# marcin119a/vae-los-angeles

Measured on AMD Instinct MI355X. Metric: training samples/sec, MultiModalVAE batch 65536, higher is better.
Workload: dtype bf16

## Files before the change

### include/mmvae_hip.h

```cpp
#ifndef MMVAE_HIP_H
#define MMVAE_HIP_H
#include <stdint.h>

#ifdef __cplusplus
extern "C" {
#endif

#define MMVAE_OK 0
#define MMVAE_ERR_ARG (-1)
#define MMVAE_ERR_DTYPE (-2)

enum { MMVAE_F32 = 0, MMVAE_BF16 = 1 };
enum { MMVAE_PREC_F32 = 0, MMVAE_PREC_BF16 = 1 };
enum { MMVAE_PRO_NONE = 0, MMVAE_PRO_BN_RELU_DROP = 1, MMVAE_PRO_BN_BWD_APPLY = 2 };
enum { MMVAE_EPI_STORE = 0, MMVAE_EPI_RELU_MASK = 1, MMVAE_EPI_BN_BWD = 2, MMVAE_EPI_LOSS_MSE = 3, MMVAE_EPI_LOSS_BCE_LOGIT = 4 };
enum { MMVAE_ACT_NONE = 0, MMVAE_ACT_RELU = 1, MMVAE_ACT_SIGMOID = 2 };

#define MMVAE_TILE 128

int mmvae_abi_version(void);
int mmvae_set_tuning(int32_t key, int32_t value);

typedef struct {
    const float* src; void* dst;
// ... 112 lines not shown
int mmvae_loss_finalize(const double* sums, float beta, float gamma, const float* beta_gamma_dev, float* out5, void* stream);

int mmvae_sigmoid_bwd(int32_t M, int32_t N, const float* g, int64_t ldg, const float* p, int64_t ldpp,
                      void* out, int32_t out_dtype, int64_t ldo, void* stream);

int mmvae_scale_if_needed(void* x, int32_t dtype, int64_t n, const float* scale_dev, void* stream);
#define MMVAE_SCALE_MAX 8
typedef struct { void* x; int64_t n; int32_t dtype; int32_t pad_; } mmvae_scale_item;
int mmvae_scale_many(const mmvae_scale_item* items_host, int32_t n_items, const float* scale_dev, void* stream);

#define MMVAE_CTR_COPIES 16384
int mmvae_noise(uint8_t* mask, int64_t n_mask, float keep_prob, float* eps, int64_t n_eps, uint64_t seed, uint64_t offset,
                uint64_t* offset_dev, int32_t advance, void* stream);
int mmvae_counter_add(uint64_t* counter_dev, uint64_t inc, void* stream);

#define MMVAE_GATHER_MAX 4
typedef struct { const void* src; void* dst; int64_t src_row_stride; int64_t dst_row_stride; int32_t row_bytes; int32_t pad_; } mmvae_gather_item;
int mmvae_gather_rows(const mmvae_gather_item* items_host, int32_t n_items, const int64_t* idx_dev, int32_t rows,
                      int64_t src_rows, void* stream);

int mmvae_rows_to_bf16(const void* src, int32_t src_dtype, int64_t ld_src, void* dst, int64_t ld_dst, int32_t rows, int32_t cols,
                       void* stream);

typedef struct { float* p; const float* g; float* m; float* v; int64_t n; } mmvae_adamw_item;
int mmvae_adamw_step(const mmvae_adamw_item* items_host, int32_t n_items, float lr, float beta1,
                     float beta2, float eps, float weight_decay, float bias_corr1, float bias_corr2, int32_t maximize,
                     uint64_t* step_dev, int32_t advance, const float* lr_dev, void* stream);

#ifdef __cplusplus
}
// ... 3 lines not shown
```

### vae-los-angeles_amd/csrc/elementwise.hip

```cpp
#include <vector>
#include "common.h"
#include "mmvae_hip.h"

namespace mm {

__global__ __launch_bounds__(256) void prep_weights_kernel(const mmvae_prep_item* __restrict__ items) {
    const mmvae_prep_item it = items[blockIdx.y];
    __shared__ float tile[32][33];
    const int tx = threadIdx.x & 31, ty = threadIdx.x >> 5;
    const int tiles_c = (it.dst_cols + 31) / 32, tiles_r = (it.dst_rows + 31) / 32;
    auto put = [&](int r, int c, float v) {
        if (it.dst_dtype == MMVAE_BF16) ((bf16*)it.dst)[(long)r * it.dst_ld + c] = (bf16)v;
        else ((float*)it.dst)[(long)r * it.dst_ld + c] = v;
    };
    for (int t = blockIdx.x; t < tiles_r * tiles_c; t += gridDim.x) {
        const int tr = t / tiles_c, tc = t - tr * tiles_c;
        if (it.transpose) {
#pragma unroll
            for (int k = 0; k < 4; ++k) {
                const int sr = tc * 32 + ty + 8 * k, sc = tr * 32 + tx;
                tile[ty + 8 * k][tx] = (sr < it.src_rows && sc < it.src_cols) ? it.src[(long)sr * it.src_ld + sc] : 0.f;
            }
            __syncthreads();
#pragma unroll
            for (int k = 0; k < 4; ++k) {
                const int r = tr * 32 + ty + 8 * k, c = tc * 32 + tx;
                if (r < it.dst_rows && c < it.dst_cols) put(r, c, tile[tx][ty + 8 * k]);
            }
            __syncthreads();
        } else {
#pragma unroll
            for (int k = 0; k < 4; ++k) {
                const int r = tr * 32 + ty + 8 * k, c = tc * 32 + tx;
                if (r < it.dst_rows && c < it.dst_cols) put(r, c, (r < it.src_rows && c < it.src_cols) ? it.src[(long)r * it.src_ld + c] : 0.f);
            }
        }
    }
}

__global__ __launch_bounds__(256) void bn_finalize_kernel(mmvae_bn_finalize_args a) {
    const int col = blockIdx.x * blockDim.x + threadIdx.x;
    if (col < a.N) {
        const double mean = a.sum[col] / a.M;
        double var = a.sumsq[col] / a.M - mean * mean;
        if (var < 0.0) var = 0.0;
        const float rstd = (float)(1.0 / sqrt(var + (double)a.eps));
        const float sc = a.gamma[col] * rstd;
        a.mean[col] = (float)mean; a.rstd[col] = rstd;
        a.scale[col] = sc; a.shift[col] = a.beta[col] - (float)mean * sc;
        if (a.running_mean) {
            a.running_mean[col] = (1.f - a.momentum) * a.running_mean[col] + a.momentum * (float)mean;
            const double unbiased = var * ((double)a.M / (double)(a.M - 1));
// ... 81 lines not shown
        }
#pragma unroll
        for (int u = 0; u < U; ++u) {
            if (r + u * dr >= (unsigned)M) break;
            float o[V];
#pragma unroll
            for (int e = 0; e < V; ++e) {
                const float xh = (yv[u][e] - mu[e]) * rs[e];
                o[e] = c0[e] * (dv[u][e] - c1[e] - xh * c2[e]);
            }
            store_vec<T, V>(d + (long)rr[u] * ldd + c, o);
        }
    }
}

__global__ __launch_bounds__(256) void embed_table_fwd_kernel(int S, int E, int L, const float* emb, const float* w_mu,
                                                               const float* b_mu, const float* w_lv, const float* b_lv, float* table) {
    for (int i = blockIdx.x * blockDim.x + threadIdx.x; i < S * 2 * L; i += gridDim.x * blockDim.x) {
        const int s = i / (2 * L), j = i % (2 * L);
        const float* w = j < L ? w_mu + (long)j * E : w_lv + (long)(j - L) * E;
        float acc = j < L ? b_mu[j] : b_lv[j - L];
        for (int e = 0; e < E; ++e) acc += emb[(long)s * E + e] * w[e];
        table[i] = acc;
    }
}

__global__ __launch_bounds__(256) void embed_table_bwd_kernel(int S, int E, int L, const float* emb, const float* w_mu,
                                                               const float* w_lv, const float* dTc, int copies, float* d_emb, float* d_w_mu,
                                                               float* d_b_mu, float* d_w_lv, float* d_b_lv) {
    const int L2 = 2 * L;
    extern __shared__ float sm[];
    float* dT = sm;
    float* sE = dT + S * L2;
    float* sW = sE + S * E;
    const int t0 = blockIdx.x * blockDim.x + threadIdx.x, nt = gridDim.x * blockDim.x;
    const int n0 = S * E, n1 = n0 + L2 * E, n2 = n1 + L2;
    auto dst_of = [&](int i) -> float* {
        if (i < n0) return d_emb + i;
        if (i < n1) { const int k = i - n0, j = k / E, e = k - j * E; return j < L ? d_w_mu + (long)j * E + e : d_w_lv + (long)(j - L) * E + e; }
// ... 413 lines not shown
            float sn, cs;
            sincosf(6.283185307179586f * u2, &sn, &cs);
            z[2 * k] = rad * cs; z[2 * k + 1] = rad * sn;
        }
        if (q * 4 + 4 <= n && (((uintptr_t)out & 15) == 0)) *(f32x4*)(out + q * 4) = f32x4{z[0], z[1], z[2], z[3]};
        else for (int k = 0; k < 4; ++k) if (q * 4 + k < n) out[q * 4 + k] = z[k];
}

__device__ __forceinline__ uint64_t ctr_read(const uint64_t* copies, unsigned L) { return copies[L % MMVAE_CTR_COPIES]; }
__device__ __forceinline__ void ctr_advance(uint64_t* copies, unsigned L, unsigned nblocks, uint64_t value) {
    __syncthreads();
    if (threadIdx.x == 0 && threadIdx.y == 0)
        for (unsigned e = L; e < MMVAE_CTR_COPIES; e += nblocks) copies[e] = value;
}

__global__ __launch_bounds__(256) void noise_kernel(uint8_t* mask, long n_mask, float* eps, long n_eps, uint32_t thresh,
                                                    uint64_t seed, uint64_t offset, uint64_t* offset_dev, uint64_t advance, int copies) {
    const uint64_t base = offset_dev ? (copies ? ctr_read(offset_dev, blockIdx.x) : *offset_dev) : 0;
    offset += base;
    const long nqm = (n_mask + 15) / 16, nqe = (n_eps + 3) / 4;
    for (long q = (long)blockIdx.x * blockDim.x + threadIdx.x; q < nqm + nqe; q += (long)gridDim.x * blockDim.x) {
        if (q < nqm) mask_quad(mask, n_mask, q, thresh, seed, offset);
        else randn_quad(eps, n_eps, q - nqm, seed, offset + (uint64_t)nqm * 4);
    }
    if (copies) ctr_advance(offset_dev, blockIdx.x, gridDim.x, base + advance);
}

__global__ void counter_add_kernel(uint64_t* ctr, uint64_t inc) { *ctr += inc; }

struct GatherBatch { mmvae_gather_item it[MMVAE_GATHER_MAX]; int n; };
__global__ __launch_bounds__(256) void gather_rows_kernel(const GatherBatch b, const int64_t* __restrict__ idx, int rows, long src_rows) {
    const int lane = threadIdx.x & 63;
    const long wave0 = ((long)blockIdx.x * blockDim.x + threadIdx.x) >> 6, nwaves = ((long)gridDim.x * blockDim.x) >> 6;
    for (long w = wave0; w < (long)rows * b.n; w += nwaves) {
        const int t = (int)(w / rows), i = (int)(w - (long)t * rows);
        const mmvae_gather_item it = b.it[t];
        long r = idx[i];
        r = r < 0 ? 0 : (r >= src_rows ? src_rows - 1 : r);
        const char* sp = (const char*)it.src + r * it.src_row_stride;
        char* dp = (char*)it.dst + (long)i * it.dst_row_stride;
// ... 79 lines not shown
static inline int grid_for(long items, int per_block = 256, int cap = 2048) {
    long g = (items + per_block - 1) / per_block;
    if (g < 1) g = 1;
    if (g > cap) g = cap;
    return (int)g;
}

}

using namespace mm;

extern "C" int mmvae_abi_version(void) { return 20; }

extern "C" int mmvae_prep_weights(const mmvae_prep_item* items_dev, int32_t n_items, void* stream) {
    if (!items_dev || n_items <= 0) return MMVAE_ERR_ARG;
    hipLaunchKernelGGL(prep_weights_kernel, dim3(160, n_items), dim3(256), 0, (hipStream_t)stream, items_dev);
    MM_CHECK_LAUNCH();
    return 0;
}

extern "C" int mmvae_bn_finalize(const mmvae_bn_finalize_args* a, void* stream) {
    if (!a || !a->sum || !a->sumsq || !a->gamma || !a->beta || !a->mean || !a->rstd || !a->scale || !a->shift) return MMVAE_ERR_ARG;
    if (a->M < 2 || a->N <= 0) return MMVAE_ERR_ARG;
    hipLaunchKernelGGL(bn_finalize_kernel, dim3((a->N + 255) / 256), dim3(256), 0, (hipStream_t)stream, *a);
    MM_CHECK_LAUNCH();
    return 0;
}

extern "C" int mmvae_bn_eval_coeffs(int32_t N, const float* gamma, const float* beta, const float* rm, const float* rv,
                                    float eps, float* scale, float* shift, float* mean, float* rstd, void* stream) {
    if (N <= 0 || !gamma || !beta || !rm || !rv || !scale || !shift) return MMVAE_ERR_ARG;
// ... 187 lines not shown
    }
    hipLaunchKernelGGL(scale_many_kernel, dim3(grid_for(nmax)), dim3(256), 0, (hipStream_t)stream, b, scale_dev);
    MM_CHECK_LAUNCH();
    return 0;
}

extern "C" int mmvae_scale_if_needed(void* x, int32_t dtype, int64_t n, const float* scale_dev, void* stream) {
    if (!x || n <= 0 || !scale_dev) return MMVAE_ERR_ARG;
    const int grid = grid_for(n);
    if (dtype == MMVAE_BF16) hipLaunchKernelGGL(scale_if_needed_kernel<bf16>, dim3(grid), dim3(256), 0, (hipStream_t)stream, (bf16*)x, n, scale_dev);
    else hipLaunchKernelGGL(scale_if_needed_kernel<float>, dim3(grid), dim3(256), 0, (hipStream_t)stream, (float*)x, n, scale_dev);
    MM_CHECK_LAUNCH();
    return 0;
}

extern "C" int mmvae_noise(uint8_t* mask, int64_t n_mask, float keep_prob, float* eps, int64_t n_eps, uint64_t seed,
                           uint64_t offset, uint64_t* offset_dev, int32_t advance, void* stream) {
    if ((n_mask > 0 && (!mask || ((uintptr_t)mask & 15))) || (n_eps > 0 && !eps) || n_mask < 0 || n_eps < 0 || n_mask + n_eps == 0 ||
        keep_prob < 0.f || keep_prob > 1.f || (advance && !offset_dev)) return MMVAE_ERR_ARG;
    const uint64_t used = (uint64_t)((n_mask + 15) / 16 * 4 + (n_eps + 3) / 4);
    const double t = (double)keep_prob * 4294967296.0;
    const uint32_t thresh = t >= 4294967295.0 ? 0xFFFFFFFFu : (uint32_t)t;
    hipLaunchKernelGGL(noise_kernel, dim3(grid_for((n_mask + 15) / 16 + (n_eps + 3) / 4)), dim3(256), 0, (hipStream_t)stream,
                       mask, n_mask, eps, n_eps, thresh, seed, offset, offset_dev, used, advance ? 1 : 0);
    MM_CHECK_LAUNCH();
    return 0;
}

extern "C" int mmvae_gather_rows(const mmvae_gather_item* items_host, int32_t n_items, const int64_t* idx_dev, int32_t rows,
                                 int64_t src_rows, void* stream) {
    if (!items_host || n_items <= 0 || n_items > MMVAE_GATHER_MAX || !idx_dev || rows <= 0 || src_rows <= 0) return MMVAE_ERR_ARG;
    GatherBatch b; b.n = n_items;
    for (int k = 0; k < n_items; ++k) {
        const mmvae_gather_item& it = items_host[k];
        if (!it.src || !it.dst || it.row_bytes <= 0 || it.row_bytes % 4 || it.src_row_stride % 4 || it.dst_row_stride % 4 ||
            ((uintptr_t)it.src & 3) || ((uintptr_t)it.dst & 3)) return MMVAE_ERR_ARG;
        b.it[k] = it;
    }
    const long waves = (long)rows * n_items;
// ... 57 lines not shown
```

### vae-los-angeles_amd/mmvae/_lib.py

```python
import ctypes as C
import os

_HERE = os.path.dirname(os.path.abspath(__file__))
LIB_PATH = os.environ.get("MMVAE_LIB_PATH") or os.path.join(_HERE, "libmmvae_hip.so")
ABI_VERSION = 20

F32, BF16 = 0, 1
PREC_F32, PREC_BF16 = 0, 1
PRO_NONE, PRO_BN_RELU_DROP, PRO_BN_BWD_APPLY = 0, 1, 2
TABLE_COPIES = 8
EPI_STORE, EPI_RELU_MASK, EPI_BN_BWD, EPI_LOSS_MSE, EPI_LOSS_BCE_LOGIT = 0, 1, 2, 3, 4
ACT_NONE, ACT_RELU, ACT_SIGMOID = 0, 1, 2
TILE = 128
TN_GROUP_MAX = 8
CTR_COPIES = 16384

i32, i64, f32, vp = C.c_int32, C.c_int64, C.c_float, C.c_void_p


class PrepItem(C.Structure):
    _fields_ = [("src", vp), ("dst", vp), ("src_rows", i32), ("src_cols", i32), ("src_ld", i64),
                ("dst_rows", i32), ("dst_cols", i32), ("dst_ld", i64), ("transpose", i32), ("dst_dtype", i32)]


# ... 68 lines not shown
                ("sums", vp),
                ("g_a", vp), ("g_a_dtype", i32), ("ld_ga", i64),
                ("g_b", vp), ("g_b_dtype", i32), ("ld_gb", i64), ("grad_b_wrt_logit", i32),
                ("g_c", vp), ("ld_gc", i64),
                ("g_mu", vp), ("g_lv", vp), ("beta_gamma_dev", vp), ("a_dtype", i32), ("b_dtype", i32)]


class GatherItem(C.Structure):
    _fields_ = [("src", vp), ("dst", vp), ("src_row_stride", i64), ("dst_row_stride", i64), ("row_bytes", i32), ("pad_", i32)]


class AdamWItem(C.Structure):
    _fields_ = [("p", vp), ("g", vp), ("m", vp), ("v", vp), ("n", i64)]


_SIGNATURES = {
    "mmvae_set_tuning": [i32, i32],
    "mmvae_prep_weights": [vp, i32, vp],
    "mmvae_gemm_nt": [C.POINTER(GemmNtArgs), vp],
    "mmvae_gemm_tn": [C.POINTER(GemmTnArgs), vp],
    "mmvae_gemm_tn_group": [vp, i32, vp],
    "mmvae_bn_finalize": [C.POINTER(BnFinalizeArgs), vp],
    "mmvae_bn_eval_coeffs": [i32, vp, vp, vp, vp, f32, vp, vp, vp, vp, vp],
    "mmvae_bn_bwd_finalize": [C.POINTER(BnBwdFinalizeArgs), vp],
    "mmvae_bn_bwd_apply": [i32, i32, i32, vp, i64, vp, i64, vp, vp, vp, vp],
    "mmvae_bn_bwd_finalize_apply": [i32, i32, i32, vp, i64, vp, i64, vp, vp, vp, vp, vp, vp, vp, i32, vp],
    "mmvae_embed_table_fwd": [i32, i32, i32, vp, vp, vp, vp, vp, vp, vp],
    "mmvae_embed_table_bwd": [i32, i32, i32, vp, vp, vp, vp, i32, vp, vp, vp, vp, vp, vp],
    "mmvae_fuse_reparam_fwd": [C.POINTER(FuseFwdArgs), vp],
    "mmvae_fuse_reparam_bwd": [C.POINTER(FuseBwdArgs), vp],
    "mmvae_vae_loss": [C.POINTER(LossArgs), vp],
    "mmvae_loss_finalize": [vp, f32, f32, vp, vp, vp],
    "mmvae_gather_rows": [vp, i32, vp, i32, i64, vp],
    "mmvae_rows_to_bf16": [vp, i32, i64, vp, i64, i32, i32, vp],
    "mmvae_sigmoid_bwd": [i32, i32, vp, i64, vp, i64, vp, i32, i64, vp],
    "mmvae_scale_if_needed": [vp, i32, i64, vp, vp],
    "mmvae_scale_many": [C.POINTER(ScaleItem), i32, vp, vp],
    "mmvae_noise": [vp, i64, f32, vp, i64, C.c_uint64, C.c_uint64, vp, i32, vp],
    "mmvae_counter_add": [vp, C.c_uint64, vp],
    "mmvae_adamw_step": [vp, i32, f32, f32, f32, f32, f32, f32, f32, i32, vp, i32, vp, vp],
}
EXPORTED = ["mmvae_abi_version"] + sorted(_SIGNATURES)

_lib = None


class MMVAELibraryError(RuntimeError):
    pass


class MMVAEArgError(RuntimeError):
    """The library refused the arguments (MMVAE_ERR_ARG / MMVAE_ERR_DTYPE) and enqueued nothing (mmvae_hip.h)."""


def load():
    global _lib
    if _lib is not None:
        return _lib
    if not os.path.exists(LIB_PATH):
        raise MMVAELibraryError(
            f"{LIB_PATH} not found: the HIP extension is required (no CPU / eager fallback). "
            "Build it with `python __graft_entry__.py` or `make -C vae-los-angeles_amd/csrc`.")
    lib = C.CDLL(LIB_PATH)
    lib.mmvae_abi_version.restype = C.c_int
    v = lib.mmvae_abi_version()
    if v != ABI_VERSION:
        raise MMVAELibraryError(f"libmmvae_hip.so ABI {v} != binding ABI {ABI_VERSION}; rebuild")
    for name, argtypes in _SIGNATURES.items():
        fn = getattr(lib, name)
        fn.restype = C.c_int
        fn.argtypes = argtypes
    _lib = lib
    return lib


def check(status, what):
    if status in (-1, -2):
        kind = "invalid argument" if status == -1 else "dtype not supported for this precision"
        raise MMVAEArgError(f"{what} failed: {kind}")
    if status != 0:
        raise RuntimeError(f"{what} failed: hipError {status}")
```

### vae-los-angeles_amd/mmvae/engine.py

```python
import os
from dataclasses import dataclass
from typing import NamedTuple, Optional

import torch

from . import ops
from . import _lib as L_
from .ops import (PREC_BF16, PREC_F32, ACT_NONE, ACT_RELU, ACT_SIGMOID, EPI_RELU_MASK, EPI_BN_BWD, DROP_P,
                  ceil_to, act_dtype, Prologue, BnBwdEpilogue, BnBwdFinalize, BnBwdApply)

_PRECISIONS = {"bf16": PREC_BF16, "fp32": PREC_F32, "f32": PREC_F32}
_default_precision = _PRECISIONS[os.environ.get("MMVAE_PRECISION", "bf16").lower()]
_TINY_DW_MAX = 16384


def set_default_precision(name):
    global _default_precision
    _default_precision = _PRECISIONS[name.lower()]


def default_precision():
    return _default_precision


class NoiseSource:

    def __init__(self):
        self._injected = None
# ... 17 lines not shown

    def offset_tensor(self, device):
        t = self._offsets.get(device)
        if t is None:
            t = self._offsets[device] = torch.zeros(L_.CTR_COPIES, dtype=torch.int64, device=device)
        return t

    def state_dict(self, device):
        t = self._offsets.get(torch.device(device) if not isinstance(device, torch.device) else device)
        return {"offset": 0 if t is None else int(t[0].item())}

    def load_state_dict(self, state, device):
        device = torch.device(device) if not isinstance(device, torch.device) else device
        self.offset_tensor(device).fill_(int(state["offset"]))

    def draw(self, B, widths, Ld, device):
        if self._injected is not None:
            masks = []
            for w in widths:
                m = self._injected[0].pop(0)
                if tuple(m.shape) != (B, w):
                    raise ValueError(f"injected mask shape {tuple(m.shape)} != {(B, w)}")
                masks.append(m.to(device=device, dtype=torch.uint8).contiguous())
            eps = None
            if Ld is not None:
                eps = self._injected[1]
                if tuple(eps.shape) != (B, Ld):
                    raise ValueError(f"injected eps shape {tuple(eps.shape)} != {(B, Ld)}")
                eps = eps.to(device=device, dtype=torch.float32).contiguous()
            return masks, eps
        segs, total = [], 0
        for w in widths:
            segs.append(total)
            total = ceil_to(total + B * w, 16)
        buf = torch.empty(total, dtype=torch.uint8, device=device) if total else None
        eps = torch.empty(B, Ld, dtype=torch.float32, device=device) if Ld is not None else None
        off = self.offset_tensor(device)
        ops.noise(buf, eps, 1.0 - DROP_P, self._seed(), 0, off, advance=True)
        return [buf[o:o + B * w].view(B, w) for o, w in zip(segs, widths)], eps


GLOBAL_NOISE = NoiseSource()


def _check_input(x, name, cols, prec):
    if x.dim() != 2 or x.shape[1] != cols:
        raise RuntimeError(f"{name}: expected shape (B, {cols}), got {tuple(x.shape)}")
    if not x.is_cuda:
        raise RuntimeError(f"{name}: the MI355X path needs CUDA/HIP tensors (got {x.device}); there is no CPU fallback")
    if x.dtype == torch.bfloat16:
        if prec != PREC_BF16:
            return x.float()
        return x if ops.is_bf16_rows(x) else ops.to_bf16_rows(x)
    if x.dtype != torch.float32:
        x = x.float()
    if x.stride(1) != 1:
        x = x.contiguous()
    return x


def zeros_pack(device, specs):
    offs, total = [], 0
    for n, dt in specs:
        offs.append(total)
        total += ceil_to(n * _ITEMSIZE[dt], 16)
    buf = torch.zeros(max(total, 16), dtype=torch.uint8, device=device)
    return [buf[o:o + n * _ITEMSIZE[dt]].view(dt) for o, (n, dt) in zip(offs, specs)]


_ITEMSIZE = {torch.float32: 4, torch.float64: 8, torch.uint8: 1, torch.int64: 8}


def carve_arena(flat, params):
    views, off = {}, 0
    for p in params:
        views[p] = flat[off:off + p.numel()].view(p.shape)
        off += p.numel()
    return views


class PrepCache:

    def __init__(self):
        self.key = self.prep = None

    def ensure(self, prec, device, params, build):
        key = (prec, str(device)) + tuple(p.data_ptr() for p in params)
        if key != self.key:
            pls = build(prec, device)
            self.prep = ops.WeightPrep(pls, device) if pls else None
            self.key = key
        if self.prep is not None:
            self.prep.run()


class BNState:

    def __init__(self, N, device):
        self.buf = torch.empty(4, N, dtype=torch.float32, device=device)
        self.mean, self.rstd, self.scale, self.shift = self.buf[0], self.buf[1], self.buf[2], self.buf[3]


class LayerSave(NamedTuple):
    q: torch.Tensor
    q_prologue: Optional[Prologue]
    y: torch.Tensor
    bn: BNState
# ... 12 lines not shown
    g_outs: list
    g_mu: torch.Tensor
    g_lv: torch.Tensor
    unit_grad: bool
    scale: Optional[torch.Tensor] = None
    armed: bool = False


@dataclass(slots=True, eq=False)
class StepZeros:
    fwd_stats: list
    loss_ws: Optional[tuple]
    arena: Optional[torch.Tensor]
    bwd_stats: list
    d_table: Optional[torch.Tensor]


@dataclass(slots=True, eq=False)
class StepState:
    prec: int
    B: int
    train: bool
    eps: Optional[torch.Tensor] = None
    logvar: Optional[torch.Tensor] = None
    n_mod: int = 0
    enc_a: Optional[list] = None
    enc_b: Optional[list] = None
    site: Optional[torch.Tensor] = None
    dec: Optional[list] = None
    zeros: Optional[StepZeros] = None
# ... 125 lines not shown
    return torch.as_strided(t, (n,), (1,))


class EmbedEncoder:

    def __init__(self, embedding, fc_mu, fc_logvar):
        self.embedding, self.fc_mu, self.fc_logvar = embedding, fc_mu, fc_logvar
        self.latent = fc_mu.out_features

    def prepare(self, prec, device):
        return []

    def params(self):
        return [self.embedding.weight, self.fc_mu.weight, self.fc_mu.bias, self.fc_logvar.weight, self.fc_logvar.bias]

    def table(self):
        emb = self.embedding.weight
        t = torch.empty(emb.shape[0], 2 * self.latent, dtype=torch.float32, device=emb.device)
        ops.embed_table_fwd(emb, self.fc_mu.weight, self.fc_mu.bias, self.fc_logvar.weight, self.fc_logvar.bias, t)
        return t

    def backward(self, d_table, grads):
        ops.embed_table_bwd(self.embedding.weight, self.fc_mu.weight, self.fc_logvar.weight, d_table,
                            grads[self.embedding.weight], grads[self.fc_mu.weight], grads[self.fc_mu.bias],
                            grads[self.fc_logvar.weight], grads[self.fc_logvar.bias])


class DecoderMLP:

    def __init__(self, linears, final_sigmoid, name="dec"):
        self.linears, self.final_sigmoid = list(linears), final_sigmoid
        self.out_dim = self.linears[-1].out_features
        self.name = name

# ... 96 lines not shown
    def early_cut(self):
        return sum(p.numel() for b in self.blocks if b not in self.decoders for p in b.params()) + sum(p.numel() for p in self._late_decoder_params())

    def _prepare(self, prec, device):
        pls = []
        for b in self.blocks:
            pls += b.prepare(prec, device)
        self.dec_stem = None
        decs = self.decoders
        if (len(decs) >= 2 and all(isinstance(d, DecoderMLP) and len(d.linears) >= 2 for d in decs)
                and all(d.linears[0].in_features == decs[0].linears[0].in_features and d.linears[0].out_features % 8 == 0 for d in decs)):
            self.dec_stem = ops.PreparedLinear([d.linears[0].weight for d in decs], [d.linears[0].bias for d in decs], prec, device)
            pls.append(self.dec_stem)
        return pls

    def zero_pack(self, device, has_a, has_b, has_site, fwd, bwd):
        widths = (self.enc_a.widths() if has_a else []) + (self.enc_b.widths() if has_b else [])
        n_sums = 2 * sum(widths)
        n_sites = self.enc_c.embedding.weight.shape[0] if has_site else 0
        n_tab = n_sites * 2 * self.latent * L_.TABLE_COPIES
        both = fwd and bwd
        fwd_sums, loss_sums, loss_out5, arena, bwd_sums, d_table = zeros_pack(device, [
            (n_sums if fwd else 0, torch.float64),
            (5 if both else 0, torch.float64),
            (5 if both else 0, torch.float32),
            (sum(p.numel() for p in self.param_list()) if bwd else 0, torch.float32),
            (n_sums if bwd else 0, torch.float64),
            (max(n_tab, 1) if bwd else 0, torch.float32)])

        def per_layer(sums):
            return [t.view(2, -1) for t in sums.split([2 * w for w in widths])]
        return StepZeros(fwd_stats=per_layer(fwd_sums) if fwd else [],
                         loss_ws=(loss_sums, loss_out5) if both else None,
                         arena=arena if bwd else None,
                         bwd_stats=per_layer(bwd_sums) if bwd else [],
                         d_table=d_table[:n_tab].view(-1, n_sites, 2 * self.latent) if bwd and has_site else None)

    def forward(self, prec, xa, xb, site, train, want_bwd=False):
        ref = xa if xa is not None else (xb if xb is not None else site)
        if not ref.is_cuda or any(p.device != ref.device for p in self.param_list()):
            raise RuntimeError(f"the MI355X path needs inputs and parameters on one CUDA/HIP device (input on {ref.device}); "
                               "there is no CPU fallback")
        with ops.pinned_stream():
            return self._forward(prec, xa, xb, site, train, train and want_bwd)

    def _forward(self, prec, xa, xb, site, train, want_bwd):
        ref = xa if xa is not None else (xb if xb is not None else site)
        dev, B = ref.device, ref.shape[0]
        self._prep.ensure(prec, dev, self.param_list(), self._prepare)
        state = StepState(prec, B, train)
        heads_a = heads_b = table = None
        Ld = self.latent
        widths_a = self.enc_a.widths() if (train and xa is not None) else []
        widths_b = self.enc_b.widths() if (train and xb is not None) else []
        n_a = len(widths_a)
        masks, eps = self.noise.draw(B, widths_a + widths_b, Ld, dev)
        zeros = self.zero_pack(dev, xa is not None, xb is not None, site is not None, fwd=True, bwd=want_bwd) if train else None
        if want_bwd:
            state.zeros = zeros
        if xa is not None:
            xa = _check_input(xa, "a", self.enc_a.in_dim, prec)
            heads_a, state.enc_a = self.enc_a.forward(prec, xa, train, masks[:n_a] if train else None,
                                                      zeros.fwd_stats[:n_a] if train else None, want_bwd=want_bwd)
        if xb is not None:
            xb = _check_input(xb.reshape(xb.shape[0], -1), "b", self.enc_b.in_dim, prec)
            heads_b, state.enc_b = self.enc_b.forward(prec, xb, train, masks[n_a:] if train else None,
                                                      zeros.fwd_stats[n_a:] if train else None, want_bwd=want_bwd)
        if site is not None:
            if site.dtype != torch.int64:
                site = site.long()
            site = site.contiguous()
            table = self.enc_c.table()
            state.site = site
        mu = torch.empty(B, Ld, dtype=torch.float32, device=dev)
        logvar = torch.empty(B, Ld, dtype=torch.float32, device=dev)
        z = torch.empty(B, ceil_to(Ld, 8), dtype=act_dtype(prec), device=dev)
        ops.fuse_reparam_fwd(B, Ld, heads_a, heads_b, table, site, eps, mu, logvar, z)
        state.eps, state.logvar = eps, logvar.detach()
        state.n_mod = (heads_a is not None) + (heads_b is not None) + (table is not None)
        outs, state.dec = [None] * len(self.decoders), [None] * len(self.decoders)
        order = sorted(range(len(self.decoders)), key=lambda i: -sum(l.weight.numel() for l in self.decoders[i].linears))
        stem = self.dec_stem
        firsts = [None] * len(self.decoders)
        if stem is not None:
            H0 = torch.empty(B, stem.N, dtype=act_dtype(prec), device=dev)
            ops.gemm_nt(prec, z, stem.w, stem.N, stem.K, H0, bias=stem.bias, act=ACT_RELU, tag="Decoders.L0.fwd")
            off = 0
# ... 90 lines not shown
```

### vae-los-angeles_amd/mmvae/ops.py

```python
import ctypes as C
from collections import namedtuple

import torch

from . import _lib as L
from ._lib import (F32, BF16, PREC_F32, PREC_BF16, PRO_NONE, PRO_BN_RELU_DROP, PRO_BN_BWD_APPLY, EPI_STORE, EPI_RELU_MASK,
                   EPI_BN_BWD, EPI_LOSS_MSE, EPI_LOSS_BCE_LOGIT, ACT_NONE, ACT_RELU, ACT_SIGMOID, TILE)

DROP_P = 0.1
BN_EPS, BN_MOMENTUM = 1e-5, 0.1


class KernelProbe:

    def __init__(self, only=None):
        self.records = {}
        self.only = only

    def wants(self, tag):
        return tag is not None and (self.only is None or tag in self.only)

    def begin(self):
        ev = torch.cuda.Event(enable_timing=True)
        ev.record(torch.cuda.current_stream())
# ... 167 lines not shown
                out.append(L.PrepItem(b.data_ptr(), self._bias_cat.data_ptr() + row * 4, 1, n, n, 1, n, n, 0, F32))
            row += n
        return out


class WeightPrep:

    def __init__(self, linears, device):
        self.linears = list(linears)
        items = [it for pl in self.linears for it in pl.items()]
        self.n = len(items)
        arr = (L.PrepItem * self.n)(*items)
        host = torch.frombuffer(bytearray(bytes(arr)), dtype=torch.uint8)
        self.table = host.to(device)

    def run(self):
        with stream_span("prep_weights", lambda: sum(6 * w.numel() for pl in self.linears for w in pl.srcs)):
            L.check(L.load().mmvae_prep_weights(self.table.data_ptr(), self.n, _stream()), "mmvae_prep_weights")


def can_keep_pro_out(prec, M, N, K, a, out):
    return (prec == PREC_BF16 and a.dtype == torch.bfloat16 and out.dtype == torch.bfloat16 and M >= 16384 and M % 128 == 0
            and N % 128 == 0 and N <= 256 and K % 64 == 0 and 64 < K <= 512 and _ld(a) % 8 == 0 and _ld(out) % 64 == 0
            and M * _ld(a) * 2 < 2 ** 31
            and a.data_ptr() % 16 == 0 and out.data_ptr() % 128 == 0)


Prologue = namedtuple("Prologue", "scale shift mask inv_keep")
BnBwdEpilogue = namedtuple("BnBwdEpilogue", "scale shift mean rstd mask inv_keep")
BnBwdFinalize = namedtuple("BnBwdFinalize", "stats gamma dgamma dbeta eval_mode")
BnBwdApply = namedtuple("BnBwdApply", "y mean rstd coef fin", defaults=(None, None))

# ... 249 lines not shown

def scale_if_needed(x, scale):
    L.check(L.load().mmvae_scale_if_needed(x.data_ptr(), _dt(x), x.numel(), scale.data_ptr(), _stream()), "mmvae_scale_if_needed")


def noise(mask, eps, keep_prob, seed, offset, offset_dev=None, advance=False):
    n_mask = 0 if mask is None else mask.numel()
    n_eps = 0 if eps is None else eps.numel()
    if advance:
        assert offset_dev is not None and offset_dev.numel() == L.CTR_COPIES and offset_dev.dtype == torch.int64
    with stream_span("noise", n_mask + 4 * n_eps):
        L.check(L.load().mmvae_noise(_p(mask), n_mask, keep_prob, _p(eps), n_eps, seed, offset, _p(offset_dev), int(advance), _stream()), "mmvae_noise")
    return (n_mask + 15) // 16 * 4 + (n_eps + 3) // 4


def dropout_mask(mask, keep_prob, seed, offset):
    return noise(mask, None, keep_prob, seed, offset)


def randn(out, seed, offset):
    return noise(None, out, 1.0, seed, offset)


def counter_add(counter, inc):
    L.check(L.load().mmvae_counter_add(counter.data_ptr(), inc, _stream()), "mmvae_counter_add")


def _gather_row(t):
    es = t.element_size()
    if t.is_contiguous():
# ... 38 lines not shown
```

Measured before the change: 51.57 million.

## Fuse step-start weight prep, zero fill, embed table, and noise into one launch

Adds a single step_begin kernel that partitions its grid among four previously separate jobs: weight prep/transposition, zeroing the workspace arena, computing the site embedding table, and drawing dropout masks and Gaussian noise. The Python forward path collects these into a StepBegin object and launches once, instead of issuing a torch.zeros plus three kernels. The goal is to cut launch overhead and serialization of small kernels at the start of each training step and let them run concurrently. In exchange the blocks are heterogeneous, the kernel pins waves-per-EU, and the noise-counter semantics depend on the noise block count.

```diff
diff --git a/include/mmvae_hip.h b/include/mmvae_hip.h
--- a/include/mmvae_hip.h
+++ b/include/mmvae_hip.h
@@ -150,6 +150,15 @@
                 uint64_t* offset_dev, int32_t advance, void* stream);
 int mmvae_counter_add(uint64_t* counter_dev, uint64_t inc, void* stream);
 
+typedef struct {
+    uint8_t* mask; int64_t n_mask; float keep_prob; float* eps; int64_t n_eps; uint64_t seed; uint64_t offset;
+    uint64_t* offset_dev; int32_t advance;
+    int32_t n_prep; const mmvae_prep_item* prep_items_dev;
+    int32_t S, E, L; const float* emb; const float* w_mu; const float* b_mu; const float* w_lv; const float* b_lv; float* table;
+    void* zero; int64_t zero_bytes;
+} mmvae_step_begin_args;
+int mmvae_step_begin(const mmvae_step_begin_args* args, void* stream);
+
 #define MMVAE_GATHER_MAX 4
 typedef struct { const void* src; void* dst; int64_t src_row_stride; int64_t dst_row_stride; int32_t row_bytes; int32_t pad_; } mmvae_gather_item;
 int mmvae_gather_rows(const mmvae_gather_item* items_host, int32_t n_items, const int64_t* idx_dev, int32_t rows,
diff --git a/vae-los-angeles_amd/csrc/elementwise.hip b/vae-los-angeles_amd/csrc/elementwise.hip
--- a/vae-los-angeles_amd/csrc/elementwise.hip
+++ b/vae-los-angeles_amd/csrc/elementwise.hip
@@ -4,8 +4,7 @@
 
 namespace mm {
 
-__global__ __launch_bounds__(256) void prep_weights_kernel(const mmvae_prep_item* __restrict__ items) {
-    const mmvae_prep_item it = items[blockIdx.y];
+__device__ __forceinline__ void prep_item_body(const mmvae_prep_item& it, int bx, int nbx) {
     __shared__ float tile[32][33];
     const int tx = threadIdx.x & 31, ty = threadIdx.x >> 5;
     const int tiles_c = (it.dst_cols + 31) / 32, tiles_r = (it.dst_rows + 31) / 32;
@@ -13,7 +12,7 @@
         if (it.dst_dtype == MMVAE_BF16) ((bf16*)it.dst)[(long)r * it.dst_ld + c] = (bf16)v;
         else ((float*)it.dst)[(long)r * it.dst_ld + c] = v;
     };
-    for (int t = blockIdx.x; t < tiles_r * tiles_c; t += gridDim.x) {
+    for (int t = bx; t < tiles_r * tiles_c; t += nbx) {
         const int tr = t / tiles_c, tc = t - tr * tiles_c;
         if (it.transpose) {
 #pragma unroll
@@ -36,6 +35,11 @@
             }
         }
     }
+}
+
+__global__ __launch_bounds__(256) void prep_weights_kernel(const mmvae_prep_item* __restrict__ items) {
+    const mmvae_prep_item it = items[blockIdx.y];
+    prep_item_body(it, blockIdx.x, gridDim.x);
 }
 
 __global__ __launch_bounds__(256) void bn_finalize_kernel(mmvae_bn_finalize_args a) {
@@ -147,15 +151,20 @@
     }
 }
 
-__global__ __launch_bounds__(256) void embed_table_fwd_kernel(int S, int E, int L, const float* emb, const float* w_mu,
-                                                               const float* b_mu, const float* w_lv, const float* b_lv, float* table) {
-    for (int i = blockIdx.x * blockDim.x + threadIdx.x; i < S * 2 * L; i += gridDim.x * blockDim.x) {
+__device__ __forceinline__ void embed_table_fwd_body(int S, int E, int L, const float* emb, const float* w_mu, const float* b_mu,
+                                                     const float* w_lv, const float* b_lv, float* table, int t0, int nt) {
+    for (int i = t0; i < S * 2 * L; i += nt) {
         const int s = i / (2 * L), j = i % (2 * L);
         const float* w = j < L ? w_mu + (long)j * E : w_lv + (long)(j - L) * E;
         float acc = j < L ? b_mu[j] : b_lv[j - L];
         for (int e = 0; e < E; ++e) acc += emb[(long)s * E + e] * w[e];
         table[i] = acc;
     }
+}
+
+__global__ __launch_bounds__(256) void embed_table_fwd_kernel(int S, int E, int L, const float* emb, const float* w_mu,
+                                                               const float* b_mu, const float* w_lv, const float* b_lv, float* table) {
+    embed_table_fwd_body(S, E, L, emb, w_mu, b_mu, w_lv, b_lv, table, blockIdx.x * blockDim.x + threadIdx.x, gridDim.x * blockDim.x);
 }
 
 __global__ __launch_bounds__(256) void embed_table_bwd_kernel(int S, int E, int L, const float* emb, const float* w_mu,
@@ -599,16 +608,55 @@
         for (unsigned e = L; e < MMVAE_CTR_COPIES; e += nblocks) copies[e] = value;
 }
 
-__global__ __launch_bounds__(256) void noise_kernel(uint8_t* mask, long n_mask, float* eps, long n_eps, uint32_t thresh,
-                                                    uint64_t seed, uint64_t offset, uint64_t* offset_dev, uint64_t advance, int copies) {
-    const uint64_t base = offset_dev ? (copies ? ctr_read(offset_dev, blockIdx.x) : *offset_dev) : 0;
-    offset += base;
-    const long nqm = (n_mask + 15) / 16, nqe = (n_eps + 3) / 4;
-    for (long q = (long)blockIdx.x * blockDim.x + threadIdx.x; q < nqm + nqe; q += (long)gridDim.x * blockDim.x) {
-        if (q < nqm) mask_quad(mask, n_mask, q, thresh, seed, offset);
-        else randn_quad(eps, n_eps, q - nqm, seed, offset + (uint64_t)nqm * 4);
-    }
-    if (copies) ctr_advance(offset_dev, blockIdx.x, gridDim.x, base + advance);
+struct NoiseJob { uint8_t* mask; long n_mask; float* eps; long n_eps; uint32_t thresh; uint64_t seed, offset; uint64_t* offset_dev; uint64_t advance; int copies; };
+__device__ __forceinline__ void noise_body(const NoiseJob& j, unsigned blk, unsigned nblk) {
+    const uint64_t base = j.offset_dev ? (j.copies ? ctr_read(j.offset_dev, blk) : *j.offset_dev) : 0;
+    const uint64_t offset = j.offset + base;
+    const long nqm = (j.n_mask + 15) / 16, nqe = (j.n_eps + 3) / 4;
+    for (long q = (long)blk * blockDim.x + threadIdx.x; q < nqm + nqe; q += (long)nblk * blockDim.x) {
+        if (q < nqm) mask_quad(j.mask, j.n_mask, q, j.thresh, j.seed, offset);
+        else randn_quad(j.eps, j.n_eps, q - nqm, j.seed, offset + (uint64_t)nqm * 4);
+    }
+    if (j.copies) ctr_advance(j.offset_dev, blk, nblk, base + j.advance);
+}
+
+__global__ __launch_bounds__(256) void noise_kernel(const NoiseJob j) { noise_body(j, blockIdx.x, gridDim.x); }
+
+constexpr int PREP_BLOCKS = 160;
+#ifndef MM_STEP_BEGIN_PREP_BLOCKS
+#define MM_STEP_BEGIN_PREP_BLOCKS 160
+#endif
+#ifndef MM_STEP_BEGIN_FILL_BLOCKS
+#define MM_STEP_BEGIN_FILL_BLOCKS 512
+#endif
+constexpr int SB_PREP_BLOCKS = MM_STEP_BEGIN_PREP_BLOCKS;
+struct StepBeginJob {
+    const mmvae_prep_item* items; int nb_prep;
+    uint4* zero; long zero_chunks; uint8_t* zero_tail; int zero_tail_bytes; int nb_fill;
+    int S, E, L; const float* emb; const float* w_mu; const float* b_mu; const float* w_lv; const float* b_lv; float* table; int nb_table;
+    NoiseJob noise; int nb_noise;
+};
+__global__ __launch_bounds__(256) __attribute__((amdgpu_waves_per_eu(8, 8))) void step_begin_kernel(const StepBeginJob a) {
+    int b = blockIdx.x;
+    if (b < a.nb_prep) {
+        const mmvae_prep_item it = a.items[b / SB_PREP_BLOCKS];
+        prep_item_body(it, b % SB_PREP_BLOCKS, SB_PREP_BLOCKS);
+        return;
+    }
+    b -= a.nb_prep;
+    if (b < a.nb_fill) {
+        const uint4 z = {0u, 0u, 0u, 0u};
+        for (long i = (long)b * 256 + threadIdx.x; i < a.zero_chunks; i += (long)a.nb_fill * 256) a.zero[i] = z;
+        if (b == 0 && (int)threadIdx.x < a.zero_tail_bytes) a.zero_tail[threadIdx.x] = 0;
+        return;
+    }
+    b -= a.nb_fill;
+    if (b < a.nb_table) {
+        embed_table_fwd_body(a.S, a.E, a.L, a.emb, a.w_mu, a.b_mu, a.w_lv, a.b_lv, a.table, b * 256 + threadIdx.x, a.nb_table * 256);
+        return;
+    }
+    b -= a.nb_table;
+    noise_body(a.noise, b, a.nb_noise);
 }
 
 __global__ void counter_add_kernel(uint64_t* ctr, uint64_t inc) { *ctr += inc; }
@@ -718,7 +766,7 @@
 
 extern "C" int mmvae_prep_weights(const mmvae_prep_item* items_dev, int32_t n_items, void* stream) {
     if (!items_dev || n_items <= 0) return MMVAE_ERR_ARG;
-    hipLaunchKernelGGL(prep_weights_kernel, dim3(160, n_items), dim3(256), 0, (hipStream_t)stream, items_dev);
+    hipLaunchKernelGGL(prep_weights_kernel, dim3(PREP_BLOCKS, n_items), dim3(256), 0, (hipStream_t)stream, items_dev);
     MM_CHECK_LAUNCH();
     return 0;
 }
@@ -936,15 +984,57 @@
     return 0;
 }
 
-extern "C" int mmvae_noise(uint8_t* mask, int64_t n_mask, float keep_prob, float* eps, int64_t n_eps, uint64_t seed,
-                           uint64_t offset, uint64_t* offset_dev, int32_t advance, void* stream) {
-    if ((n_mask > 0 && (!mask || ((uintptr_t)mask & 15))) || (n_eps > 0 && !eps) || n_mask < 0 || n_eps < 0 || n_mask + n_eps == 0 ||
-        keep_prob < 0.f || keep_prob > 1.f || (advance && !offset_dev)) return MMVAE_ERR_ARG;
+static bool noise_args_ok(const uint8_t* mask, int64_t n_mask, float keep_prob, const float* eps, int64_t n_eps, const uint64_t* offset_dev, int32_t advance) {
+    return !((n_mask > 0 && (!mask || ((uintptr_t)mask & 15))) || (n_eps > 0 && !eps) || n_mask < 0 || n_eps < 0 || n_mask + n_eps == 0 ||
+             keep_prob < 0.f || keep_prob > 1.f || (advance && !offset_dev));
+}
+
+static NoiseJob noise_job(uint8_t* mask, int64_t n_mask, float keep_prob, float* eps, int64_t n_eps, uint64_t seed, uint64_t offset,
+                          uint64_t* offset_dev, int32_t advance) {
     const uint64_t used = (uint64_t)((n_mask + 15) / 16 * 4 + (n_eps + 3) / 4);
     const double t = (double)keep_prob * 4294967296.0;
     const uint32_t thresh = t >= 4294967295.0 ? 0xFFFFFFFFu : (uint32_t)t;
+    return NoiseJob{mask, (long)n_mask, eps, (long)n_eps, thresh, seed, offset, offset_dev, used, advance ? 1 : 0};
+}
+
+extern "C" int mmvae_noise(uint8_t* mask, int64_t n_mask, float keep_prob, float* eps, int64_t n_eps, uint64_t seed,
+                           uint64_t offset, uint64_t* offset_dev, int32_t advance, void* stream) {
+    if (!noise_args_ok(mask, n_mask, keep_prob, eps, n_eps, offset_dev, advance)) return MMVAE_ERR_ARG;
     hipLaunchKernelGGL(noise_kernel, dim3(grid_for((n_mask + 15) / 16 + (n_eps + 3) / 4)), dim3(256), 0, (hipStream_t)stream,
-                       mask, n_mask, eps, n_eps, thresh, seed, offset, offset_dev, used, advance ? 1 : 0);
+                       noise_job(mask, n_mask, keep_prob, eps, n_eps, seed, offset, offset_dev, advance));
+    MM_CHECK_LAUNCH();
+    return 0;
+}
+
+#ifndef MM_STEP_BEGIN_NOISE_BLOCKS
+#define MM_STEP_BEGIN_NOISE_BLOCKS 1536
+#endif
+
+extern "C" int mmvae_step_begin(const mmvae_step_begin_args* a, void* stream) {
+    if (!a) return MMVAE_ERR_ARG;
+    if (a->n_mask < 0 || a->n_eps < 0 || a->n_prep < 0 || a->zero_bytes < 0) return MMVAE_ERR_ARG;
+    const bool has_noise = a->n_mask + a->n_eps > 0, has_prep = a->n_prep > 0, has_table = a->table != nullptr, has_fill = a->zero_bytes > 0;
+    if (!has_noise && !has_prep && !has_table && !has_fill) return MMVAE_ERR_ARG;
+    if (has_noise && !noise_args_ok(a->mask, a->n_mask, a->keep_prob, a->eps, a->n_eps, a->offset_dev, a->advance)) return MMVAE_ERR_ARG;
+    if (has_prep && (!a->prep_items_dev || (long)a->n_prep * SB_PREP_BLOCKS > (1L << 20))) return MMVAE_ERR_ARG;
+    if (has_table && (a->S <= 0 || a->E <= 0 || a->L <= 0 || !a->emb || !a->w_mu || !a->b_mu || !a->w_lv || !a->b_lv)) return MMVAE_ERR_ARG;
+    if (has_fill && (!a->zero || ((uintptr_t)a->zero & 15))) return MMVAE_ERR_ARG;
+    StepBeginJob j = {};
+    if (has_prep) { j.items = a->prep_items_dev; j.nb_prep = a->n_prep * SB_PREP_BLOCKS; }
+    if (has_fill) {
+        j.zero = (uint4*)a->zero; j.zero_chunks = a->zero_bytes / 16;
+        j.zero_tail = (uint8_t*)a->zero + j.zero_chunks * 16; j.zero_tail_bytes = (int)(a->zero_bytes % 16);
+        j.nb_fill = grid_for(j.zero_chunks, 256 * 4, MM_STEP_BEGIN_FILL_BLOCKS);
+    }
+    if (has_table) {
+        j.S = a->S; j.E = a->E; j.L = a->L; j.emb = a->emb; j.w_mu = a->w_mu; j.b_mu = a->b_mu; j.w_lv = a->w_lv; j.b_lv = a->b_lv; j.table = a->table;
+        j.nb_table = grid_for((long)a->S * 2 * a->L, 256, 64);
+    }
+    if (has_noise) {
+        j.noise = noise_job(a->mask, a->n_mask, a->keep_prob, a->eps, a->n_eps, a->seed, a->offset, a->offset_dev, a->advance);
+        j.nb_noise = grid_for((a->n_mask + 15) / 16 + (a->n_eps + 3) / 4, 256, MM_STEP_BEGIN_NOISE_BLOCKS);
+    }
+    hipLaunchKernelGGL(step_begin_kernel, dim3(j.nb_prep + j.nb_fill + j.nb_table + j.nb_noise), dim3(256), 0, (hipStream_t)stream, j);
     MM_CHECK_LAUNCH();
     return 0;
 }
diff --git a/vae-los-angeles_amd/mmvae/_lib.py b/vae-los-angeles_amd/mmvae/_lib.py
--- a/vae-los-angeles_amd/mmvae/_lib.py
+++ b/vae-los-angeles_amd/mmvae/_lib.py
@@ -106,6 +106,14 @@
     _fields_ = [("p", vp), ("g", vp), ("m", vp), ("v", vp), ("n", i64)]
 
 
+class StepBeginArgs(C.Structure):
+    _fields_ = [("mask", vp), ("n_mask", i64), ("keep_prob", f32), ("eps", vp), ("n_eps", i64), ("seed", C.c_uint64), ("offset", C.c_uint64),
+                ("offset_dev", vp), ("advance", i32),
+                ("n_prep", i32), ("prep_items_dev", vp),
+                ("S", i32), ("E", i32), ("L", i32), ("emb", vp), ("w_mu", vp), ("b_mu", vp), ("w_lv", vp), ("b_lv", vp), ("table", vp),
+                ("zero", vp), ("zero_bytes", i64)]
+
+
 _SIGNATURES = {
     "mmvae_set_tuning": [i32, i32],
     "mmvae_prep_weights": [vp, i32, vp],
@@ -130,6 +138,7 @@
     "mmvae_scale_many": [C.POINTER(ScaleItem), i32, vp, vp],
     "mmvae_noise": [vp, i64, f32, vp, i64, C.c_uint64, C.c_uint64, vp, i32, vp],
     "mmvae_counter_add": [vp, C.c_uint64, vp],
+    "mmvae_step_begin": [C.POINTER(StepBeginArgs), vp],
     "mmvae_adamw_step": [vp, i32, f32, f32, f32, f32, f32, f32, f32, i32, vp, i32, vp, vp],
 }
 EXPORTED = ["mmvae_abi_version"] + sorted(_SIGNATURES)
@@ -159,7 +168,9 @@
     if v != ABI_VERSION:
         raise MMVAELibraryError(f"libmmvae_hip.so ABI {v} != binding ABI {ABI_VERSION}; rebuild")
     for name, argtypes in _SIGNATURES.items():
-        fn = getattr(lib, name)
+        fn = getattr(lib, name, None)
+        if fn is None:
+            raise MMVAELibraryError(f"libmmvae_hip.so lacks {name}; rebuild")
         fn.restype = C.c_int
         fn.argtypes = argtypes
     _lib = lib
diff --git a/vae-los-angeles_amd/mmvae/engine.py b/vae-los-angeles_amd/mmvae/engine.py
--- a/vae-los-angeles_amd/mmvae/engine.py
+++ b/vae-los-angeles_amd/mmvae/engine.py
@@ -12,6 +12,7 @@
 _PRECISIONS = {"bf16": PREC_BF16, "fp32": PREC_F32, "f32": PREC_F32}
 _default_precision = _PRECISIONS[os.environ.get("MMVAE_PRECISION", "bf16").lower()]
 _TINY_DW_MAX = 16384
+SIDE_BY_SIDE = True
 
 
 def set_default_precision(name):
@@ -59,7 +60,7 @@
         device = torch.device(device) if not isinstance(device, torch.device) else device
         self.offset_tensor(device).fill_(int(state["offset"]))
 
-    def draw(self, B, widths, Ld, device):
+    def draw(self, B, widths, Ld, device, begin=None):
         if self._injected is not None:
             masks = []
             for w in widths:
@@ -81,7 +82,8 @@
         buf = torch.empty(total, dtype=torch.uint8, device=device) if total else None
         eps = torch.empty(B, Ld, dtype=torch.float32, device=device) if Ld is not None else None
         off = self.offset_tensor(device)
-        ops.noise(buf, eps, 1.0 - DROP_P, self._seed(), 0, off, advance=True)
+        draw = ops.noise if begin is None else begin.noise
+        draw(buf, eps, 1.0 - DROP_P, self._seed(), 0, off, advance=True)
         return [buf[o:o + B * w].view(B, w) for o, w in zip(segs, widths)], eps
 
 
@@ -104,13 +106,14 @@
     return x
 
 
-def zeros_pack(device, specs):
+def zeros_pack(device, specs, fill=True):
     offs, total = [], 0
     for n, dt in specs:
         offs.append(total)
         total += ceil_to(n * _ITEMSIZE[dt], 16)
-    buf = torch.zeros(max(total, 16), dtype=torch.uint8, device=device)
-    return [buf[o:o + n * _ITEMSIZE[dt]].view(dt) for o, (n, dt) in zip(offs, specs)]
+    buf = (torch.zeros if fill else torch.empty)(max(total, 16), dtype=torch.uint8, device=device)
+    views = [buf[o:o + n * _ITEMSIZE[dt]].view(dt) for o, (n, dt) in zip(offs, specs)]
+    return views if fill else (views, buf)
 
 
 _ITEMSIZE = {torch.float32: 4, torch.float64: 8, torch.uint8: 1, torch.int64: 8}
@@ -129,13 +132,13 @@
     def __init__(self):
         self.key = self.prep = None
 
-    def ensure(self, prec, device, params, build):
+    def ensure(self, prec, device, params, build, run=True):
         key = (prec, str(device)) + tuple(p.data_ptr() for p in params)
         if key != self.key:
             pls = build(prec, device)
             self.prep = ops.WeightPrep(pls, device) if pls else None
             self.key = key
-        if self.prep is not None:
+        if run and self.prep is not None:
             self.prep.run()
 
 
@@ -178,6 +181,7 @@
     arena: Optional[torch.Tensor]
     bwd_stats: list
     d_table: Optional[torch.Tensor]
+    unfilled: Optional[torch.Tensor] = None
 
 
 @dataclass(slots=True, eq=False)
@@ -333,10 +337,10 @@
     def params(self):
         return [self.embedding.weight, self.fc_mu.weight, self.fc_mu.bias, self.fc_logvar.weight, self.fc_logvar.bias]
 
-    def table(self):
+    def table(self, begin=None):
         emb = self.embedding.weight
         t = torch.empty(emb.shape[0], 2 * self.latent, dtype=torch.float32, device=emb.device)
-        ops.embed_table_fwd(emb, self.fc_mu.weight, self.fc_mu.bias, self.fc_logvar.weight, self.fc_logvar.bias, t)
+        (ops.embed_table_fwd if begin is None else begin.table)(emb, self.fc_mu.weight, self.fc_mu.bias, self.fc_logvar.weight, self.fc_logvar.bias, t)
         return t
 
     def backward(self, d_table, grads):
@@ -463,19 +467,20 @@
             pls.append(self.dec_stem)
         return pls
 
-    def zero_pack(self, device, has_a, has_b, has_site, fwd, bwd):
+    def zero_pack(self, device, has_a, has_b, has_site, fwd, bwd, fill=True):
         widths = (self.enc_a.widths() if has_a else []) + (self.enc_b.widths() if has_b else [])
         n_sums = 2 * sum(widths)
         n_sites = self.enc_c.embedding.weight.shape[0] if has_site else 0
         n_tab = n_sites * 2 * self.latent * L_.TABLE_COPIES
         both = fwd and bwd
-        fwd_sums, loss_sums, loss_out5, arena, bwd_sums, d_table = zeros_pack(device, [
+        views = zeros_pack(device, [
             (n_sums if fwd else 0, torch.float64),
             (5 if both else 0, torch.float64),
             (5 if both else 0, torch.float32),
             (sum(p.numel() for p in self.param_list()) if bwd else 0, torch.float32),
             (n_sums if bwd else 0, torch.float64),
-            (max(n_tab, 1) if bwd else 0, torch.float32)])
+            (max(n_tab, 1) if bwd else 0, torch.float32)], fill=fill)
+        (fwd_sums, loss_sums, loss_out5, arena, bwd_sums, d_table), unfilled = views if not fill else (views, None)
 
         def per_layer(sums):
             return [t.view(2, -1) for t in sums.split([2 * w for w in widths])]
@@ -483,7 +488,8 @@
                          loss_ws=(loss_sums, loss_out5) if both else None,
                          arena=arena if bwd else None,
                          bwd_stats=per_layer(bwd_sums) if bwd else [],
-                         d_table=d_table[:n_tab].view(-1, n_sites, 2 * self.latent) if bwd and has_site else None)
+                         d_table=d_table[:n_tab].view(-1, n_sites, 2 * self.latent) if bwd and has_site else None,
+                         unfilled=unfilled)
 
     def forward(self, prec, xa, xb, site, train, want_bwd=False):
         ref = xa if xa is not None else (xb if xb is not None else site)
@@ -496,17 +502,27 @@
     def _forward(self, prec, xa, xb, site, train, want_bwd):
         ref = xa if xa is not None else (xb if xb is not None else site)
         dev, B = ref.device, ref.shape[0]
-        self._prep.ensure(prec, dev, self.param_list(), self._prepare)
+        begin = ops.StepBegin() if SIDE_BY_SIDE else None
+        self._prep.ensure(prec, dev, self.param_list(), self._prepare, run=begin is None)
+        if begin is not None and self._prep.prep is not None:
+            begin.prep(self._prep.prep)
         state = StepState(prec, B, train)
         heads_a = heads_b = table = None
         Ld = self.latent
         widths_a = self.enc_a.widths() if (train and xa is not None) else []
         widths_b = self.enc_b.widths() if (train and xb is not None) else []
         n_a = len(widths_a)
-        masks, eps = self.noise.draw(B, widths_a + widths_b, Ld, dev)
-        zeros = self.zero_pack(dev, xa is not None, xb is not None, site is not None, fwd=True, bwd=want_bwd) if train else None
+        masks, eps = self.noise.draw(B, widths_a + widths_b, Ld, dev, begin=begin)
+        zeros = self.zero_pack(dev, xa is not None, xb is not None, site is not None, fwd=True, bwd=want_bwd, fill=begin is None) if train else None
         if want_bwd:
             state.zeros = zeros
+        if begin is not None:
+            if zeros is not None:
+                begin.zero(zeros.unfilled)
+                zeros.unfilled = None
+            if site is not None:
+                table = self.enc_c.table(begin)
+            begin.launch()
         if xa is not None:
             xa = _check_input(xa, "a", self.enc_a.in_dim, prec)
             heads_a, state.enc_a = self.enc_a.forward(prec, xa, train, masks[:n_a] if train else None,
@@ -519,7 +535,8 @@
             if site.dtype != torch.int64:
                 site = site.long()
             site = site.contiguous()
-            table = self.enc_c.table()
+            if begin is None:
+                table = self.enc_c.table()
             state.site = site
         mu = torch.empty(B, Ld, dtype=torch.float32, device=dev)
         logvar = torch.empty(B, Ld, dtype=torch.float32, device=dev)
diff --git a/vae-los-angeles_amd/mmvae/ops.py b/vae-los-angeles_amd/mmvae/ops.py
--- a/vae-los-angeles_amd/mmvae/ops.py
+++ b/vae-los-angeles_amd/mmvae/ops.py
@@ -205,8 +205,11 @@
         host = torch.frombuffer(bytearray(bytes(arr)), dtype=torch.uint8)
         self.table = host.to(device)
 
+    def nbytes(self):
+        return sum(6 * w.numel() for pl in self.linears for w in pl.srcs)
+
     def run(self):
-        with stream_span("prep_weights", lambda: sum(6 * w.numel() for pl in self.linears for w in pl.srcs)):
+        with stream_span("prep_weights", self.nbytes):
             L.check(L.load().mmvae_prep_weights(self.table.data_ptr(), self.n, _stream()), "mmvae_prep_weights")
 
 
@@ -486,6 +489,52 @@
     return (n_mask + 15) // 16 * 4 + (n_eps + 3) // 4
 
 
+class StepBegin:
+
+    def __init__(self):
+        self.args = L.StepBeginArgs()
+        self.nbytes = 0
+        self._keep = []
+
+    def noise(self, mask, eps, keep_prob, seed, offset, offset_dev=None, advance=False):
+        a = self.args
+        n_mask = 0 if mask is None else mask.numel()
+        n_eps = 0 if eps is None else eps.numel()
+        if advance:
+            assert offset_dev is not None and offset_dev.numel() == L.CTR_COPIES and offset_dev.dtype == torch.int64
+        a.mask, a.n_mask, a.keep_prob, a.eps, a.n_eps = _p(mask), n_mask, keep_prob, _p(eps), n_eps
+        a.seed, a.offset, a.offset_dev, a.advance = seed, offset, _p(offset_dev), int(advance)
+        self.nbytes += n_mask + 4 * n_eps
+        self._keep += [mask, eps, offset_dev]
+        return (n_mask + 15) // 16 * 4 + (n_eps + 3) // 4
+
+    def prep(self, weight_prep):
+        self.args.n_prep, self.args.prep_items_dev = weight_prep.n, weight_prep.table.data_ptr()
+        self.nbytes += weight_prep.nbytes()
+        self._keep.append(weight_prep)
+
+    def table(self, emb, w_mu, b_mu, w_lv, b_lv, table):
+        a = self.args
+        (a.S, a.E), a.L = emb.shape, w_mu.shape[0]
+        a.emb, a.w_mu, a.b_mu, a.w_lv, a.b_lv, a.table = (t.data_ptr() for t in (emb, w_mu, b_mu, w_lv, b_lv, table))
+        self.nbytes += 4 * (emb.numel() + w_mu.numel() + w_lv.numel() + b_mu.numel() + b_lv.numel() + table.numel())
+        self._keep += [emb, w_mu, b_mu, w_lv, b_lv, table]
+
+    def zero(self, buf):
+        assert buf.is_contiguous() and buf.data_ptr() % 16 == 0
+        self.args.zero, self.args.zero_bytes = buf.data_ptr(), buf.numel() * buf.element_size()
+        self.nbytes += self.args.zero_bytes
+        self._keep.append(buf)
+
+    def launch(self):
+        a = self.args
+        if a.n_mask + a.n_eps == 0 and a.n_prep == 0 and not a.table and a.zero_bytes == 0:
+            return
+        with stream_span("step_begin", self.nbytes):
+            L.check(L.load().mmvae_step_begin(C.byref(a), _stream()), "mmvae_step_begin")
+        self._keep.clear()
+
+
 def dropout_mask(mask, keep_prob, seed, offset):
     return noise(mask, None, keep_prob, seed, offset)
 
```

Result: no change. 51.74 million, median of 4 (+0.3%).
